# sumansamui/CMOOP_Audio_Processing

Hardware: AMD Instinct MI355X
Metric: candidate-net evals/hour (pop=40, GSC-v2) (higher is better)
Workload: dtype f32

## Files before the change

cmoop_audio_processing_amd/csrc/gemm.hip:

```cpp
#include "kernels.h"
#include <hip/hip_ext.h>
#include <cstdlib>
#include <mutex>
#include <string>
#include <type_traits>

namespace cmoop {

typedef __bf16 bf16x8 __attribute__((ext_vector_type(8)));
typedef unsigned u32x4 __attribute__((ext_vector_type(4)));

typedef __bf16 bf16x2 __attribute__((ext_vector_type(2)));

template <int NP>
__device__ __forceinline__ void split_pair(const float x, const float y, unsigned (&w)[NP]) {
    if constexpr (NP == 1) {
        w[0] = __builtin_bit_cast(unsigned, __builtin_convertvector((f32x2){x, y}, bf16x2));
    } else {
        const unsigned ux = __float_as_uint(x), uy = __float_as_uint(y);
        w[0] = __builtin_amdgcn_perm(uy, ux, 0x07060302u);
        const float rx = x - __uint_as_float(ux & 0xFFFF0000u), ry = y - __uint_as_float(uy & 0xFFFF0000u);
        const unsigned vx = __float_as_uint(rx), vy = __float_as_uint(ry);
        w[1] = __builtin_amdgcn_perm(vy, vx, 0x07060302u);
        const float sx = rx - __uint_as_float(vx & 0xFFFF0000u), sy = ry - __uint_as_float(vy & 0xFFFF0000u);
// ... 493 lines not shown
        for (int c = cbeg; c < nchunks; ++c) {
            const int buf = (c - cbeg) & 1;
            if (c + 1 < nchunks) load_chunk(c + 1, ra0, rb0);
            compute(buf);
            if (c + 1 < nchunks) store_chunk(buf ^ 1, ra0, rb0);
            __syncthreads();
        }
    }

    const int N = g.Cout;
    if (pslab) {
#pragma unroll
        for (int rt = 0; rt < RT; ++rt)
#pragma unroll
            for (int r = 0; r < 4; ++r)
#pragma unroll
                for (int ct = 0; ct < CT; ++ct)
                    pslab[(wrow + rt * 16 + q * 4 + r) * BN + wcol + ct * 16 + lr] = acc[rt][ct][r];
        continue;
    }
    if (slab) {
        float* Pz = slab + (size_t)blockIdx.z * g.M * N;
#pragma unroll
        for (int rt = 0; rt < RT; ++rt)
#pragma unroll
            for (int r = 0; r < 4; ++r) {
                const int row = m0 + wrow + rt * 16 + q * 4 + r;
                if (row >= g.M) continue;
#pragma unroll
                for (int ct = 0; ct < CT; ++ct) {
                    const int col = n0 + wcol + ct * 16 + lr;
                    if (col < N) Pz[(size_t)row * N + col] = acc[rt][ct][r];
                }
            }
        continue;
    }
    float csum[CT], csq[CT], bias_v[CT];
#pragma unroll
    for (int ct = 0; ct < CT; ++ct) {
        csum[ct] = 0.f; csq[ct] = 0.f;
        const int col = n0 + wcol + ct * 16 + lr;
        bias_v[ct] = (e.bias && col < N) ? e.bias[col] : 0.f;
    }
    const bool whole = m0 + BM <= g.M && (N % BN) == 0 && e.out_stride == 1;
    const uint32_t e_lane = (uint32_t)((m0 + wrow + q * 4) * N + n0 + wcol + lr) * 4u;
    const __amdgpu_buffer_rsrc_t yrs = __builtin_amdgcn_make_buffer_rsrc(Y, 0, g.M * N * 4, 0x00020000);
    if (whole && !e.dropout && !e.mask && !e.accumulate) {
        auto store_all = [&](auto relu_c, auto stats_c) {
#pragma unroll
            for (int rt = 0; rt < RT; ++rt)
#pragma unroll
                for (int r = 0; r < 4; ++r) {
                    const int soff = (rt * 16 + r) * N * 4;
#pragma unroll
                    for (int ct = 0; ct < CT; ++ct) {
                        float v = acc[rt][ct][r] + bias_v[ct];
                        if constexpr (decltype(relu_c)::value) v = fmaxf(v, 0.f);
                        __builtin_amdgcn_raw_buffer_store_b32(__float_as_uint(v), yrs, (int)(e_lane + ct * 64), soff, 0);
                        if constexpr (decltype(stats_c)::value) { csum[ct] += v; csq[ct] += v * v; }
                    }
                }
        };
        using T1 = std::integral_constant<bool, true>;
        using T0 = std::integral_constant<bool, false>;
        if (e.relu) { if (e.stats) store_all(T1{}, T1{}); else store_all(T1{}, T0{}); }
        else        { if (e.stats) store_all(T0{}, T1{}); else store_all(T0{}, T0{}); }
    } else if (whole && e.mask && !e.dropout && !e.relu && !e.bias && !e.stats) {
        const __amdgpu_buffer_rsrc_t mrs = __builtin_amdgcn_make_buffer_rsrc(const_cast<float*>(e.mask), 0, g.M * N * 4, 0x00020000);
#pragma unroll
        for (int rt = 0; rt < RT; ++rt) {
            float mk[4][CT], old[4][CT];
#pragma unroll
            for (int r = 0; r < 4; ++r)
#pragma unroll
                for (int ct = 0; ct < CT; ++ct) {
                    const int soff = (rt * 16 + r) * N * 4;
                    mk[r][ct] = __uint_as_float(__builtin_amdgcn_raw_buffer_load_b32(mrs, (int)(e_lane + ct * 64), soff, 0));
                    old[r][ct] = e.accumulate ? __uint_as_float(__builtin_amdgcn_raw_buffer_load_b32(yrs, (int)(e_lane + ct * 64), soff, 0)) : 0.f;
                }
#pragma unroll
            for (int r = 0; r < 4; ++r)
#pragma unroll
                for (int ct = 0; ct < CT; ++ct) {
                    const int soff = (rt * 16 + r) * N * 4;
                    float v = (mk[r][ct] > 0.f) ? acc[rt][ct][r] * e.mask_scale : 0.f;
                    if (e.accumulate) v += old[r][ct];
                    __builtin_amdgcn_raw_buffer_store_b32(__float_as_uint(v), yrs, (int)(e_lane + ct * 64), soff, 0);
                }
        }
    } else {
#pragma unroll
    for (int rt = 0; rt < RT; ++rt) {
#pragma unroll
        for (int r = 0; r < 4; ++r) {
            const int row = m0 + wrow + rt * 16 + q * 4 + r;
            if (row >= g.M) continue;
            size_t rbase;
            if (e.out_stride == 1) {
                rbase = (size_t)row * N;
            } else {
                int b = row / g.OHW, rr = row - b * g.OHW;
                int oh = rr / g.OW, ow = rr - oh * g.OW;
                rbase = ((size_t)(b * e.OHf + oh * e.out_stride) * e.OWf + ow * e.out_stride) * N;
            }
#pragma unroll
            for (int ct = 0; ct < CT; ++ct) {
                const int col = n0 + wcol + ct * 16 + lr;
                if (col >= N) continue;
                float v = acc[rt][ct][r] + bias_v[ct];
                if (e.relu) v = fmaxf(v, 0.f);
                const size_t off = rbase + col;
                if (e.dropout) {
                    uint32_t u24 = fmix32(e.drop_prefix ^ (uint32_t)((size_t)row * N + col)) >> 8;
                    v = (u24 >= e.drop_thr) ? v * e.drop_scale : 0.f;
                }
                if (e.mask) v = (e.mask[off] > 0.f) ? v * e.mask_scale : 0.f;
                if (e.accumulate) v += Y[off];
                Y[off] = v;
                csum[ct] += v;
                csq[ct] += v * v;
            }
        }
    }
    }
    if (e.stats) {
        float* red = PLANES ? reinterpret_cast<float*>(&Ah[0][0]) : &As[0][0];
#pragma unroll
        for (int ct = 0; ct < CT; ++ct) {
            csum[ct] += __shfl_xor(csum[ct], 16, 64);
            csq[ct] += __shfl_xor(csq[ct], 16, 64);
            csum[ct] += __shfl_xor(csum[ct], 32, 64);
            csq[ct] += __shfl_xor(csq[ct], 32, 64);
            if (q == 0) {
                const int c = wcol + ct * 16 + lr;
                red[((wave / WN) * BN + c) * 2] = csum[ct];
                red[((wave / WN) * BN + c) * 2 + 1] = csq[ct];
            }
        }
        __syncthreads();
        if (t < BN && n0 + t < N) {
            float a = 0.f, b = 0.f;
#pragma unroll
            for (int w = 0; w < WM; ++w) { a += red[(w * BN + t) * 2]; b += red[(w * BN + t) * 2 + 1]; }
            e.stats[((size_t)mtile * 2) * N + n0 + t] = a;
            e.stats[((size_t)mtile * 2 + 1) * N + n0 + t] = b;
        }
    }
    }
}

struct HaloDev {
    int WP, rows_max, VH;
    uint32_t wp_magic, wp_shift, vh_magic, vh_shift;
};
__host__ __device__ constexpr int halo_nst(int bm) { return bm == 256 ? 11 : 9; }
static bool halo_geometry(const ConvGeom& cg, HaloDev* hd, size_t* lds_bytes);
static size_t halo_balanced_slab_floats(const ConvGeom& cg, int* L_out);

template <int KS, int BM, int BN, int WM, bool BAL = false>
__global__ __launch_bounds__(256, 2) void halo_fwd_kernel(const float* __restrict__ X, const float* __restrict__ Wt,
                                                          float* __restrict__ Y, GeomDev g, EpiDev e, HaloDev h,
                                                          float* __restrict__ slab) {
    constexpr int WN = 4 / WM, RT = BM / WM / 16, CT = BN / WN / 16, R = KS / 2, T = KS * KS;
    constexpr int PITCH = 24;
    constexpr int NST = halo_nst(BM);
    static_assert(RT >= 1 && CT >= 1, "tile too small for the wave layout");
    extern __shared__ __attribute__((aligned(16))) float halo[];

    const int t = threadIdx.x;
    const int ncc = g.Cin >> 4;
    const int upt = ncc * KS;
    int u = 0, uend = 1;
    if constexpr (BAL) {
        const int U = ((g.M + BM - 1) / BM) * ((g.Cout + BN - 1) / BN) * upt;
        u = blockIdx.x * e.bal_L;
        uend = min(U, u + e.bal_L);
    }
    while (u < uend) {
    int mtile, ntile, c_lo = 0, c_hi = upt;
    float* pslab = nullptr;
    if constexpr (BAL) {
        const int nt = (g.Cout + BN - 1) / BN;
        const int t0 = u / upt;
        c_lo = u - t0 * upt;
        c_hi = min(upt, c_lo + (uend - u));
        mtile = t0 / nt; ntile = t0 - mtile * nt;
        const int seg = c_lo == 0 ? 0 : (int)blockIdx.x - (t0 * upt) / e.bal_L;
        pslab = slab + ((size_t)t0 * e.bal_segmax + seg) * (BM * BN);
        u += c_hi - c_lo;
        __syncthreads();
    } else {
        u = uend;
        mtile = blockIdx.x;
        const int nwg = gridDim.x, xcd = mtile & 7, idx = mtile >> 3;
        const int qn = nwg >> 3, rn = nwg & 7;
        mtile = (xcd < rn ? xcd * (qn + 1) : rn * (qn + 1) + (xcd - rn) * qn) + idx;
        ntile = blockIdx.y;
    }
    const int m0 = mtile * BM, n0 = ntile * BN;
    const int wave = t >> 6, lane = t & 63, lr = lane & 15, q = lane >> 4;
    const int wrow = (wave / WN) * (BM / WM), wcol = (wave % WN) * (BN / WN);

    auto vrow = [&](int m, int& x) {
        const int b = fastdiv(m, g.ohw_magic, g.ohw_shift), r = m - b * g.OHW;
        const int y = fastdiv(r, g.ow_magic, g.ow_shift);
        x = r - y * g.OW;
        return b * h.VH + y;
    };
    int xdummy;
    const int vbase = vrow(m0, xdummy);
    const int vlast = vrow(min(m0 + BM, g.M) - 1, xdummy);
    const int items = (vlast - vbase + 1 + 2 * R) * h.WP * 4;

    const __amdgpu_buffer_rsrc_t xr = __builtin_amdgcn_make_buffer_rsrc(
        const_cast<float*>(X), 0, (int)((uint32_t)g.B * g.H * g.W << g.cshift) * 4, 0x00020000);
    const __amdgpu_buffer_rsrc_t wr = __builtin_amdgcn_make_buffer_rsrc(const_cast<float*>(Wt), 0, g.Cout * g.K * 4, 0x00020000);
    uint32_t s_voff[NST];
#pragma unroll
    for (int it = 0; it < NST; ++it) {
        const int i = t + 256 * it, pix = i >> 2, j = i & 3;
        const int hy = fastdiv(pix, h.wp_magic, h.wp_shift), hx = pix - hy * h.WP;
        const int v = vbase - R + hy, vc = max(v, 0);
        const int b = fastdiv(vc, h.vh_magic, h.vh_shift), y = vc - b * h.VH;
        const bool ok = i < items && v >= 0 && b < g.B && y < g.H && hx >= R && hx < g.W + R;
        s_voff[it] = ok ? (uint32_t)(((((b * g.H + y) * g.W + hx - R) << g.cshift) + 4 * j) * 4) : 0xFFFFFFFFu;
    }
    float* const st_dst = halo + (t >> 2) * PITCH + (t & 3) * 4;
    f32x4 st[NST];
    auto stage_load = [&](int cc) {
#pragma unroll
        for (int it = 0; it < NST; ++it)
            st[it] = __builtin_bit_cast(f32x4, __builtin_amdgcn_raw_buffer_load_b128(xr, (int)s_voff[it], cc * 64, 0));
    };
    auto stage_store = [&]() {
#pragma unroll
        for (int it = 0; it < NST; ++it)
            if (t + 256 * it < items) *reinterpret_cast<f32x4*>(st_dst + it * 64 * PITCH) = st[it];
    };

    const float* a_ptr[RT];
#pragma unroll
    for (int rt = 0; rt < RT; ++rt) {
        int x;
        const int v = vrow(min(m0 + wrow + rt * 16 + lr, g.M - 1), x);
        a_ptr[rt] = halo + ((v - vbase) * h.WP + x) * PITCH + 4 * q;
    }
    uint32_t b_voff[CT];
#pragma unroll
    for (int ct = 0; ct < CT; ++ct) {
        const int col = n0 + wcol + ct * 16 + lr;
        b_voff[ct] = col < g.Cout ? (uint32_t)(col * g.K + 4 * q) * 4u : 0xFFFFFFFFu;
    }
    const int wp_f = h.WP * PITCH;
    auto load_b = [&](int cc, int tap, f32x4 (&b)[CT]) {
        const int soff = ((tap << g.cshift) + cc * 16) * 4;
#pragma unroll
        for (int ct = 0; ct < CT; ++ct)
            b[ct] = __builtin_bit_cast(f32x4, __builtin_amdgcn_raw_buffer_load_b128(wr, (int)b_voff[ct], soff, 0));
    };

    f32x4 acc[RT][CT];
#pragma unroll
    for (int i = 0; i < RT; ++i)
#pragma unroll
        for (int j = 0; j < CT; ++j) acc[i][j] = f32x4{0.f, 0.f, 0.f, 0.f};

    if constexpr (BAL) {
        int cc = c_lo / KS, ky = c_lo - cc * KS;
        f32x4 ac[RT], bc[CT];
        stage_load(cc);
        load_b(cc, ky * KS, bc);
        stage_store();
        __syncthreads();
#pragma unroll
        for (int rt = 0; rt < RT; ++rt) ac[rt] = *reinterpret_cast<const f32x4*>(a_ptr[rt] + ky * wp_f);
        for (int c = c_lo; c < c_hi; ++c) {
            const bool last_unit = c + 1 == c_hi, new_cc = ky == KS - 1;
            const int nky = new_cc ? 0 : ky + 1, ncc2 = new_cc ? cc + 1 : cc;
            if (new_cc && !last_unit) stage_load(cc + 1);
#pragma unroll
            for (int kx = 0; kx < KS; ++kx) {
                f32x4 an[RT], bn[CT];
#pragma unroll
                for (int ct = 0; ct < CT; ++ct) bn[ct] = bc[ct];
                if (kx + 1 < KS) {
                    load_b(cc, ky * KS + kx + 1, bn);
#pragma unroll
                    for (int rt = 0; rt < RT; ++rt)
                        an[rt] = *reinterpret_cast<const f32x4*>(a_ptr[rt] + ky * wp_f + (kx + 1) * PITCH);
                } else if (!last_unit) {
                    load_b(ncc2, nky * KS, bn);
                    if (!new_cc) {
#pragma unroll
                        for (int rt = 0; rt < RT; ++rt) an[rt] = *reinterpret_cast<const f32x4*>(a_ptr[rt] + nky * wp_f);
                    }
                }
                __builtin_amdgcn_s_setprio(1);
#pragma unroll
                for (int j = 0; j < 4; ++j)
#pragma unroll
                    for (int rt = 0; rt < RT; ++rt)
#pragma unroll
                        for (int ct = 0; ct < CT; ++ct)
                            acc[rt][ct] = __builtin_amdgcn_mfma_f32_16x16x4f32(ac[rt][j], bc[ct][j], acc[rt][ct], 0, 0, 0);
                __builtin_amdgcn_s_setprio(0);
#pragma unroll
                for (int ct = 0; ct < CT; ++ct) bc[ct] = bn[ct];
                if (kx + 1 < KS || (!last_unit && !new_cc)) {
#pragma unroll
                    for (int rt = 0; rt < RT; ++rt) ac[rt] = an[rt];
                } else if (!last_unit) {
                    __syncthreads();
                    stage_store();
                    __syncthreads();
#pragma unroll
                    for (int rt = 0; rt < RT; ++rt) ac[rt] = *reinterpret_cast<const f32x4*>(a_ptr[rt]);
                }
            }
            ky = nky; cc = ncc2;
        }
#pragma unroll
        for (int rt = 0; rt < RT; ++rt)
#pragma unroll
            for (int r = 0; r < 4; ++r)
#pragma unroll
                for (int ct = 0; ct < CT; ++ct)
                    pslab[(wrow + rt * 16 + q * 4 + r) * BN + wcol + ct * 16 + lr] = acc[rt][ct][r];
        continue;
    } else {
    f32x4 ac[RT], bc[CT];
    stage_load(0);
    load_b(0, 0, bc);
    stage_store();
    __syncthreads();
#pragma unroll
    for (int rt = 0; rt < RT; ++rt) ac[rt] = *reinterpret_cast<const f32x4*>(a_ptr[rt]);

    for (int cc = 0; cc < ncc; ++cc) {
        const bool more = cc + 1 < ncc;
#pragma unroll
        for (int tap = 0; tap < T; ++tap) {
            f32x4 an[RT], bn[CT];
#pragma unroll
            for (int ct = 0; ct < CT; ++ct) bn[ct] = bc[ct];
            if (tap + 1 < T) {
                load_b(cc, tap + 1, bn);
                const int ky = (tap + 1) / KS, kx = (tap + 1) % KS;
#pragma unroll
                for (int rt = 0; rt < RT; ++rt)
                    an[rt] = *reinterpret_cast<const f32x4*>(a_ptr[rt] + ky * wp_f + kx * PITCH);
            } else if (more) {
                load_b(cc + 1, 0, bn);
            }
            if (tap == T - 2 && more) stage_load(cc + 1);
            __builtin_amdgcn_s_setprio(1);
#pragma unroll
            for (int j = 0; j < 4; ++j)
#pragma unroll
                for (int rt = 0; rt < RT; ++rt)
#pragma unroll
                    for (int ct = 0; ct < CT; ++ct)
                        acc[rt][ct] = __builtin_amdgcn_mfma_f32_16x16x4f32(ac[rt][j], bc[ct][j], acc[rt][ct], 0, 0, 0);
            __builtin_amdgcn_s_setprio(0);
#pragma unroll
            for (int ct = 0; ct < CT; ++ct) bc[ct] = bn[ct];
            if (tap + 1 < T) {
#pragma unroll
                for (int rt = 0; rt < RT; ++rt) ac[rt] = an[rt];
            } else if (more) {
                __syncthreads();
                stage_store();
                __syncthreads();
#pragma unroll
                for (int rt = 0; rt < RT; ++rt) ac[rt] = *reinterpret_cast<const f32x4*>(a_ptr[rt]);
            }
        }
    }

    }

    const int N = g.Cout;
    float csum[CT], csq[CT], bias_v[CT];
#pragma unroll
    for (int ct = 0; ct < CT; ++ct) {
        csum[ct] = 0.f; csq[ct] = 0.f;
        const int col = n0 + wcol + ct * 16 + lr;
        bias_v[ct] = (e.bias && col < N) ? e.bias[col] : 0.f;
    }
    const bool whole = m0 + BM <= g.M && (N % BN) == 0;
    const uint32_t e_lane = (uint32_t)((m0 + wrow + q * 4) * N + n0 + wcol + lr) * 4u;
    const __amdgpu_buffer_rsrc_t yrs = __builtin_amdgcn_make_buffer_rsrc(Y, 0, g.M * N * 4, 0x00020000);
    if (whole && !e.dropout && !e.mask && !e.accumulate) {
        auto store_all = [&](auto relu_c, auto stats_c) {
#pragma unroll
            for (int rt = 0; rt < RT; ++rt)
#pragma unroll
                for (int r = 0; r < 4; ++r) {
                    const int soff = (rt * 16 + r) * N * 4;
#pragma unroll
                    for (int ct = 0; ct < CT; ++ct) {
                        float v = acc[rt][ct][r] + bias_v[ct];
                        if constexpr (decltype(relu_c)::value) v = fmaxf(v, 0.f);
                        __builtin_amdgcn_raw_buffer_store_b32(__float_as_uint(v), yrs, (int)(e_lane + ct * 64), soff, 0);
                        if constexpr (decltype(stats_c)::value) { csum[ct] += v; csq[ct] += v * v; }
                    }
                }
        };
        using T1 = std::integral_constant<bool, true>;
        using T0 = std::integral_constant<bool, false>;
        if (e.relu) { if (e.stats) store_all(T1{}, T1{}); else store_all(T1{}, T0{}); }
        else        { if (e.stats) store_all(T0{}, T1{}); else store_all(T0{}, T0{}); }
    } else if (whole && e.mask && !e.dropout && !e.relu && !e.bias && !e.stats) {
        const __amdgpu_buffer_rsrc_t mrs = __builtin_amdgcn_make_buffer_rsrc(const_cast<float*>(e.mask), 0, g.M * N * 4, 0x00020000);
#pragma unroll
        for (int rt = 0; rt < RT; ++rt) {
            float mk[4][CT], old[4][CT];
#pragma unroll
            for (int r = 0; r < 4; ++r)
#pragma unroll
                for (int ct = 0; ct < CT; ++ct) {
                    const int soff = (rt * 16 + r) * N * 4;
                    mk[r][ct] = __uint_as_float(__builtin_amdgcn_raw_buffer_load_b32(mrs, (int)(e_lane + ct * 64), soff, 0));
                    old[r][ct] = e.accumulate ? __uint_as_float(__builtin_amdgcn_raw_buffer_load_b32(yrs, (int)(e_lane + ct * 64), soff, 0)) : 0.f;
                }
#pragma unroll
            for (int r = 0; r < 4; ++r)
#pragma unroll
                for (int ct = 0; ct < CT; ++ct) {
                    const int soff = (rt * 16 + r) * N * 4;
                    float v = (mk[r][ct] > 0.f) ? acc[rt][ct][r] * e.mask_scale : 0.f;
                    if (e.accumulate) v += old[r][ct];
                    __builtin_amdgcn_raw_buffer_store_b32(__float_as_uint(v), yrs, (int)(e_lane + ct * 64), soff, 0);
                }
        }
    } else {
#pragma unroll
    for (int rt = 0; rt < RT; ++rt) {
#pragma unroll
        for (int r = 0; r < 4; ++r) {
            const int row = m0 + wrow + rt * 16 + q * 4 + r;
            if (row >= g.M) continue;
            const size_t rbase = (size_t)row * N;
#pragma unroll
            for (int ct = 0; ct < CT; ++ct) {
                const int col = n0 + wcol + ct * 16 + lr;
                if (col >= N) continue;
                float v = acc[rt][ct][r] + bias_v[ct];
                if (e.relu) v = fmaxf(v, 0.f);
                const size_t off = rbase + col;
                if (e.dropout) {
                    uint32_t u24 = fmix32(e.drop_prefix ^ (uint32_t)((size_t)row * N + col)) >> 8;
                    v = (u24 >= e.drop_thr) ? v * e.drop_scale : 0.f;
                }
                if (e.mask) v = (e.mask[off] > 0.f) ? v * e.mask_scale : 0.f;
                if (e.accumulate) v += Y[off];
                Y[off] = v;
                csum[ct] += v;
                csq[ct] += v * v;
            }
        }
    }
    }
    if (e.stats) {
        __syncthreads();
        float* red = halo;
#pragma unroll
        for (int ct = 0; ct < CT; ++ct) {
            csum[ct] += __shfl_xor(csum[ct], 16, 64);
            csq[ct] += __shfl_xor(csq[ct], 16, 64);
            csum[ct] += __shfl_xor(csum[ct], 32, 64);
            csq[ct] += __shfl_xor(csq[ct], 32, 64);
            if (q == 0) {
                const int c = wcol + ct * 16 + lr;
                red[((wave / WN) * BN + c) * 2] = csum[ct];
                red[((wave / WN) * BN + c) * 2 + 1] = csq[ct];
            }
        }
        __syncthreads();
        if (t < BN && n0 + t < N) {
            float a = 0.f, b = 0.f;
#pragma unroll
            for (int w = 0; w < WM; ++w) { a += red[(w * BN + t) * 2]; b += red[(w * BN + t) * 2 + 1]; }
            e.stats[((size_t)mtile * 2) * N + n0 + t] = a;
            e.stats[((size_t)mtile * 2 + 1) * N + n0 + t] = b;
        }
    }
    }
}

struct BalDev { int bm, bn, nt, chunks, L, segmax; };

template <int VEC>
__global__ __launch_bounds__(256) void splitk_combine_kernel(const float* __restrict__ P, float* __restrict__ Y, GeomDev g,
                                                             EpiDev e, int splits, BalDev bal) {
    const int N = g.Cout;
    const size_t total = (size_t)g.M * N;
    for (size_t i = ((size_t)blockIdx.x * 256 + threadIdx.x) * VEC; i < total; i += (size_t)gridDim.x * 256 * VEC) {
        const int row = (int)(i / N), col = (int)(i - (size_t)row * N);
        float v[VEC];
#pragma unroll
        for (int j = 0; j < VEC; ++j) v[j] = 0.f;
        if (bal.L > 0) {
            const int mt = row / bal.bm, ntl = col / bal.bn;
            const int tile = mt * bal.nt + ntl;
            const int first = (tile * bal.chunks) / bal.L;
            const int nseg = ((tile + 1) * bal.chunks + bal.L - 1) / bal.L - first;
            const float* src = P + (size_t)tile * bal.segmax * (bal.bm * bal.bn) + (size_t)(row - mt * bal.bm) * bal.bn + (col - ntl * bal.bn);
            for (int z = 0; z < nseg; ++z) {
                if constexpr (VEC == 4) {
                    const f32x4 p = *reinterpret_cast<const f32x4*>(src + (size_t)z * (bal.bm * bal.bn));
                    v[0] += p[0]; v[1] += p[1]; v[2] += p[2]; v[3] += p[3];
                } else {
                    v[0] += src[(size_t)z * (bal.bm * bal.bn)];
                }
            }
        } else
        for (int z = 0; z < splits; ++z) {
            if constexpr (VEC == 4) {
                const f32x4 p = *reinterpret_cast<const f32x4*>(P + (size_t)z * total + i);
                v[0] += p[0]; v[1] += p[1]; v[2] += p[2]; v[3] += p[3];
            } else {
                v[0] += P[(size_t)z * total + i];
            }
        }
        size_t off = i;
        if (e.out_stride != 1) {
            int b = fastdiv(row, g.ohw_magic, g.ohw_shift), rr = row - b * g.OHW;
            int oh = fastdiv(rr, g.ow_magic, g.ow_shift), ow = rr - oh * g.OW;
            off = ((size_t)(b * e.OHf + oh * e.out_stride) * e.OWf + ow * e.out_stride) * N + col;
        }
#pragma unroll
        for (int j = 0; j < VEC; ++j) {
            float x = v[j];
            if (e.bias) x += e.bias[col + j];
            if (e.relu) x = fmaxf(x, 0.f);
            if (e.dropout) {
                uint32_t u24 = fmix32(e.drop_prefix ^ (uint32_t)(i + j)) >> 8;
                x = (u24 >= e.drop_thr) ? x * e.drop_scale : 0.f;
            }
            if (e.mask) x = (e.mask[off + j] > 0.f) ? x * e.mask_scale : 0.f;
            if (e.accumulate) x += Y[off + j];
            v[j] = x;
        }
        if constexpr (VEC == 4) *reinterpret_cast<f32x4*>(Y + off) = f32x4{v[0], v[1], v[2], v[3]};
        else Y[off] = v[0];
    }
}

template <class... KA, class... A>
static void launch_timed(void (*kernel)(KA...), dim3 grid, size_t lds, hipStream_t s, const GemmTiming* tm, A&&... args) {
    if (tm && tm->start && tm->ext) {
        hipExtLaunchKernelGGL(kernel, grid, dim3(256), (uint32_t)lds, s, tm->start, tm->stop, 0, static_cast<KA>(args)...);
    } else {
        if (tm && tm->start) CMOOP_HIP(hipEventRecord(tm->start, s));
        hipLaunchKernelGGL(kernel, grid, dim3(256), lds, s, static_cast<KA>(args)...);
        if (tm && tm->start) CMOOP_HIP(hipEventRecord(tm->stop, s));
    }
}

template <int BM, int BN, int BK, int WM, int MODE = 0>
static void launch_fwd_t(const float* X, const float* Wt, float* Y, const GeomDev& g, const EpiDev& e_in, hipStream_t s,
                         const GemmTiming* tm, float* slab, int splits, int balanced_wgs = 0, const uint2* rowtab = nullptr,
                         int tab_rows = 0) {
    EpiDev e = e_in;
    dim3 grid(cdiv(g.M, BM), cdiv(g.Cout, BN), splits);
    const int nchunks = cdiv(g.K, BK);
    int cps = cdiv(nchunks, splits);
    float* sl = splits > 1 ? slab : nullptr;
    BalDev bal{BM, BN, cdiv(g.Cout, BN), nchunks, 0, 0};
    if (balanced_wgs > 0) {
        const long units = (long)grid.x * grid.y * nchunks;
        bal.L = (int)((units + balanced_wgs - 1) / balanced_wgs);
        bal.segmax = cdiv(nchunks, bal.L) + 1;
        e.bal_L = bal.L; e.bal_segmax = bal.segmax;
        grid = dim3((unsigned)((units + bal.L - 1) / bal.L), 1, 1);
        sl = slab;
        splits = 2;
    }
    launch_timed(igemm_fwd_kernel<BM, BN, BK, WM, MODE>, grid, 0, s, tm, X, Wt, Y, g, e, sl, cps, rowtab, tab_rows);
    CMOOP_HIP(hipGetLastError());
    if (splits > 1) {
        const size_t total = (size_t)g.M * g.Cout;
        if (g.Cout % 4 == 0) {
            const unsigned gridc = (unsigned)std::min<size_t>((total / 4 + 255) / 256, 4096);
            hipLaunchKernelGGL(splitk_combine_kernel<4>, dim3(gridc), dim3(256), 0, s, slab, Y, g, e, splits, bal);
        } else {
            const unsigned gridc = (unsigned)std::min<size_t>((total + 255) / 256, 4096);
            hipLaunchKernelGGL(splitk_combine_kernel<1>, dim3(gridc), dim3(256), 0, s, slab, Y, g, e, splits, bal);
        }
        CMOOP_HIP(hipGetLastError());
    }
}

static int fill_waves(long base, int max_mult, int resident, double first_thr = 0.85) {
    for (const double thr : {first_thr, 0.85}) {
        for (int m = 1; m <= max_mult; ++m) {
            const long blocks = base * m;
            const long waves = (blocks + resident - 1) / resident;
            const double u = (double)blocks / (double)(waves * resident);
            if (blocks >= resident / 2 && u >= thr) return m;
        }
    }
    int best = 1;
    double best_u = 0.0;
    for (int m = 1; m <= max_mult; ++m) {
        const long blocks = base * m;
        const long waves = (blocks + resident - 1) / resident;
        const double u = (double)blocks / (double)(waves * resident);
        if (u > best_u) { best_u = u; best = m; }
    }
    return best;
}

static inline int resident_wgs_128(int bn) { return 256 * (bn >= 64 ? 2 : 3); }

static size_t balanced_slab_floats(int M, int N, int K, int bk, int bn, int* wgs_out) {
    if (bk != 32) return 0;
    const long tiles = (long)cdiv(M, 128) * cdiv(N, bn);
    static const int mult = [] { const char* v = std::getenv("CMOOP_BALANCED_MULT"); const int m = v ? std::atoi(v) : 1; return (m == 2 || m == 4) ? m : 1; }();
    const int chunks = cdiv(K, 32), W = resident_wgs_128(bn) * mult;
    if (tiles > W || tiles * chunks < 8l * W) return 0;
    const int L = (int)((tiles * chunks + W - 1) / W);
    if (wgs_out) *wgs_out = W;
    return (size_t)tiles * (cdiv(chunks, L) + 1) * 128 * bn;
}

static void pick_tile(int M, int N, int K, int bk, size_t ws_floats, int* bm, int* bn, int* splits, int* balanced_wgs) {
    const int bn_small = N <= 16 ? 16 : (N <= 32 ? 32 : 64);
    const int bn_big = N > 64 ? 128 : bn_small;
    *splits = 1;
    *balanced_wgs = 0;
    long blocks = (long)cdiv(M, 128) * cdiv(N, bn_big);
    const long fill = std::max(32l, (long)(384 * par_scale()));
    if (blocks >= fill) { *bm = 128; *bn = bn_big; return; }
    const int nchunks = cdiv(K, bk);
    static const bool balanced_on = [] { const char* v = std::getenv("CMOOP_BALANCED"); return !(v && v[0] == '0'); }();
    if (balanced_on) {
        int W = 0;
        const size_t need = balanced_slab_floats(M, N, K, bk, bn_big, &W);
        if (need > 0 && need <= ws_floats) { *bm = 128; *bn = bn_big; *balanced_wgs = W; return; }
    }
    if (nchunks >= (M <= 512 ? 4 : 16) && ws_floats > 0) {
        const int min_chunks = M <= 512 ? 2 : 8;
        int sp = (int)std::min<long>(cdiv((int)(1024 * par_scale()), (int)blocks), nchunks / min_chunks);
        sp = std::min(sp, 32);
        if (sp > 1) sp = fill_waves(blocks, sp, std::max(32, (int)(512 * par_scale())));
        while (sp > 1 && (size_t)sp * M * N > ws_floats) --sp;
        if (sp > 1) {
            const int cps = cdiv(nchunks, sp);
            sp = cdiv(nchunks, cps);
            *bm = 128; *bn = bn_big; *splits = sp;
            return;
        }
    }
    blocks = (long)cdiv(M, 128) * cdiv(N, bn_small);
    if (blocks >= fill) { *bm = 128; *bn = bn_small; return; }
    *bm = 64; *bn = bn_small;
}

size_t igemm_splitk_workspace(const ConvGeom& g) {
    const int M = g.M(), N = g.Cout;
    const int bn_big = N > 64 ? 128 : (N <= 16 ? 16 : (N <= 32 ? 32 : 64));
    const long blocks = (long)cdiv(M, 128) * cdiv(N, bn_big);
    if (blocks >= 384) return 0;
    const int sp = std::min(32, cdiv(1024, (int)blocks));
    return std::max(std::max((size_t)sp * M * N, balanced_slab_floats(M, N, g.K(), g.Cin % 32 == 0 ? 32 : 16, bn_big, nullptr)),
                    halo_balanced_slab_floats(g, nullptr));
}

static size_t halo_balanced_slab_floats(const ConvGeom& cg, int* L_out) {
    static const bool on = [] { const char* v = std::getenv("CMOOP_HALO_BAL"); return !(v && v[0] == '0'); }();
    if (!on || cg.Cout % 64 != 0 || !halo_geometry(cg, nullptr, nullptr)) return 0;
    const long tiles = (long)cdiv(cg.M(), 128) * (cg.Cout / 64);
    const int upt = (cg.Cin / 16) * cg.KH;
    const long units = tiles * upt;
    if (tiles >= 1024 || units < 512l * 2 * cg.KH) return 0;
    const int L = (int)((units + 511) / 512);
    if (L_out) *L_out = L;
    return (size_t)tiles * (cdiv(upt, L) + 1) * 128 * 64;
}

struct FwdChoice {
    int mode, bm, bn, splits, balanced_wgs, flags;
    bool bk32_tile, use_dma, stats, halo;
    int ks, halo_L;
    int code() const { return mode * 100000000 + bm * 100000 + bn * 100 + (halo ? ks + (halo_L > 0 ? 50 : 0) : (bk32_tile ? 32 : 16)); }
};

static inline int halo_bm(int cout) { return cout >= 64 ? 128 : 256; }
static bool halo_geometry(const ConvGeom& cg, HaloDev* hd, size_t* lds_bytes) {
    const int ks = cg.KH, R = ks / 2;
    if (cg.KH != cg.KW || (ks != 3 && ks != 5) || cg.stride != 1 || cg.OH != cg.H || cg.OW != cg.W) return false;
    if (cg.pad_t != R || cg.pad_l != R || cg.Cin % 16 != 0) return false;
    if (cg.Cout % 64 != 0 && cg.Cout != 32 && cg.Cout != 16) return false;
    const int bm = halo_bm(cg.Cout);
    const int wp = (cg.W + ks - 1 + 7) / 8 * 8;
    const int span = (bm - 2 + cg.W) / cg.W + 1 + ((bm - 1) / (cg.H * cg.W) + 1) * R;
    const int rows = span + 2 * R;
    if (rows * wp * 4 > halo_nst(bm) * 256) return false;
    const size_t lds = (size_t)rows * wp * 24 * sizeof(float);
    if (lds > 64 * 1024) return false;
    if (hd) {
        hd->WP = wp; hd->rows_max = rows; hd->VH = cg.H + R;
        fastdiv_init(wp, &hd->wp_magic, &hd->wp_shift);
        fastdiv_init(cg.H + R, &hd->vh_magic, &hd->vh_shift);
    }
    if (lds_bytes) *lds_bytes = lds;
    return true;
}

void halo_rows_bound_and_need(const ConvGeom& cg, int* bound, int* need, int* items_cap) {
    HaloDev hd;
    size_t lds = 0;
    *bound = *need = *items_cap = 0;
    if (!halo_geometry(cg, &hd, &lds)) return;
    const int R = cg.KH / 2, bm = halo_bm(cg.Cout), M = cg.M(), VH = cg.H + R;
    auto vrow = [&](int m) { const int b = m / (cg.H * cg.W), r = m - b * cg.H * cg.W; return b * VH + r / cg.W; };
    int worst = 0;
    for (int m0 = 0; m0 < M; m0 += bm) worst = std::max(worst, vrow(std::min(m0 + bm, M) - 1) - vrow(m0) + 1 + 2 * R);
    *bound = hd.rows_max; *need = worst; *items_cap = halo_nst(bm) * 256 / (hd.WP * 4);
}

static size_t halo_lds_for_occupancy(size_t lds, long wgs, int occ_env) {
    auto fill = [&](long slots) { return (double)wgs / (double)(((wgs + slots - 1) / slots) * slots); };
    const bool better = wgs <= 1536 && fill(512) > fill(768) + 0.05;
    const bool two = occ_env < 0 ? better : (occ_env == 2 || (occ_env != 3 && lds <= 53 * 1024 && better));
    return two ? std::max(lds, (size_t)55 * 1024) : lds;
}

static FwdChoice choose_fwd(const ConvGeom& cg, const GemmEpilogue& ep, size_t ws_floats, bool want_stats, bool have_rowtab) {
    FwdChoice c;
    const int M = cg.M(), N = cg.Cout, K = cg.K();
    c.mode = resolve_mode(ep.mode);
    const bool bk32 = c.mode != GEMM_FP32 || (cg.Cin % 32 == 0);
    pick_tile(M, N, K, bk32 ? 32 : 16, ws_floats, &c.bm, &c.bn, &c.splits, &c.balanced_wgs);
    c.stats = want_stats && c.splits == 1 && !c.balanced_wgs && ep.out_stride == 1 && !ep.accumulate;
    c.bk32_tile = c.mode != GEMM_FP32 ||
                  (bk32 && !(c.bm == 128 && c.bn == 64 && c.splits == 1 && !c.balanced_wgs && (long)cdiv(M, 128) * cdiv(N, 64) >= 1024));
    static const int dma_env = [] { const char* v = std::getenv("CMOOP_DMA"); return v ? std::atoi(v) : 1; }();
    c.use_dma = dma_env && c.mode == GEMM_FP32 && (cg.Cin % 32 == 0) && cg.KH * cg.KW <= 32 && c.bk32_tile && c.bm == 128 && c.bn == 32;
    if (c.use_dma) c.mode = GEMM_FP32_DMA;
    const int bk = c.bk32_tile ? 32 : 16;
    static const bool halo_env = [] { const char* v = std::getenv("CMOOP_HALO"); return !(v && v[0] == '0'); }();
    c.ks = cg.KH;
    c.halo = halo_env && (c.mode == GEMM_FP32 || c.mode == GEMM_FP32_DMA) && c.bm == 128 && c.splits == 1 && !c.balanced_wgs && ep.out_stride == 1 &&
             halo_geometry(cg, nullptr, nullptr);
    c.halo_L = 0;
    if (c.halo) {
        c.mode = GEMM_FP32_HALO; c.use_dma = false;
        c.bm = halo_bm(cg.Cout);
        c.bn = std::min(cg.Cout, 64);
    } else if (halo_env && (c.mode == GEMM_FP32 || c.mode == GEMM_FP32_DMA) && c.bm == 128 && (c.splits > 1 || c.balanced_wgs) && ep.out_stride == 1) {
        int L = 0;
        const size_t need = halo_balanced_slab_floats(cg, &L);
        if (need > 0 && need <= ws_floats) {
            c.halo = true; c.halo_L = L; c.mode = GEMM_FP32_HALO; c.use_dma = false; c.stats = false;
            c.bm = 128; c.bn = 64; c.splits = 1; c.balanced_wgs = 512;
        }
    }
    c.flags = (c.splits > 1 ? GEMM_FLAG_SPLITK : 0) | (c.stats ? GEMM_FLAG_STATS : 0) | (c.balanced_wgs ? GEMM_FLAG_BALANCED : 0) |
              ((!c.halo && have_rowtab && (cg.Cin % bk) == 0 && cg.KH * cg.KW <= 32) ? GEMM_FLAG_ROWTAB : 0);
    return c;
}

int igemm_fwd_plan(const ConvGeom& g, const GemmEpilogue& ep, size_t ws_floats, bool want_stats, bool have_rowtab, int* flags_out) {
    igemm_check_range(g);
    CMOOP_REQUIRE(ilog2_exact(g.Cin) >= 4, "implicit GEMM needs C_in a power of two >= 16");
    const FwdChoice c = choose_fwd(g, ep, ws_floats, want_stats, have_rowtab);
    if (flags_out) *flags_out = c.flags;
    return c.code();
}

int launch_igemm_fwd(const float* X, const float* Wt, float* Y, const ConvGeom& cg, const GemmEpilogue& ep,
                     hipStream_t s, const GemmTiming* tm, float* splitk_ws, size_t splitk_ws_floats, int* stats_blocks,
                     const void* rowtab_v, int tab_rows, int* flags_out) {
    if (stats_blocks) *stats_blocks = 0;
    if (flags_out) *flags_out = 0;
    const uint2* rowtab = static_cast<const uint2*>(rowtab_v);
    GeomDev g = to_dev(cg);
    if (g.M == 0) return 0;
    EpiDev e;
    e.bias = ep.bias; e.mask = ep.mask; e.mask_scale = ep.mask_scale; e.relu = ep.relu;
    e.accumulate = ep.accumulate; e.out_stride = ep.out_stride; e.OHf = ep.OHf; e.OWf = ep.OWf;
    e.dropout = ep.dropout; e.drop_prefix = ep.drop_prefix; e.drop_thr = ep.drop_thr; e.drop_scale = ep.drop_scale;
    if (e.out_stride > 1)
        CMOOP_REQUIRE((int64_t)g.B * e.OHf * e.OWf * g.Cout < (1ll << 29), "scattered output too large");
    const FwdChoice ch = choose_fwd(cg, ep, splitk_ws ? splitk_ws_floats : 0, ep.stats != nullptr && stats_blocks != nullptr, rowtab != nullptr);
    const int mode = ch.mode == GEMM_FP32_DMA ? (int)GEMM_FP32 : ch.mode;
    const int bm = ch.bm, bn = ch.bn, splits = ch.splits, balanced_wgs = ch.balanced_wgs;
    const bool bk32_tile = ch.bk32_tile, use_dma = ch.use_dma;
    e.bal_L = 0; e.bal_segmax = 0;
    e.stats = ch.stats ? ep.stats : nullptr;
    if (e.stats) *stats_blocks = cdiv(g.M, bm);
    if (flags_out) *flags_out = ch.flags;
    if (ch.halo) {
        HaloDev hd;
        size_t lds = 0;
        CMOOP_REQUIRE(halo_geometry(cg, &hd, &lds), "halo kernel chosen for a geometry it does not accept");
        dim3 grid(cdiv(g.M, bm), cdiv(g.Cout, bn));
        BalDev bal{bm, bn, cdiv(g.Cout, bn), (cg.Cin / 16) * cg.KH, ch.halo_L, 0};
        if (ch.halo_L > 0) {
            bal.segmax = cdiv(bal.chunks, bal.L) + 1;
            e.bal_L = bal.L; e.bal_segmax = bal.segmax;
            const long units = (long)grid.x * grid.y * bal.chunks;
            grid = dim3((unsigned)((units + bal.L - 1) / bal.L), 1, 1);
            lds = std::max(lds, (size_t)55 * 1024);
        }
        static const int occ_env = [] { const char* v = std::getenv("CMOOP_HALO_OCC"); const int o = v ? std::atoi(v) : 0; return o == 2 || o == 3 ? o : 0; }();
        lds = halo_lds_for_occupancy(lds, (long)grid.x * grid.y, occ_env);
        auto run = [&](auto kernel) { launch_timed(kernel, grid, lds, s, tm, X, Wt, Y, g, e, hd, splitk_ws); };
#define CMOOP_HALO_KS(KS_)                                                                     \
        do {                                                                                   \
            if (ch.halo_L > 0) run(halo_fwd_kernel<KS_, 128, 64, 2, true>);                    \
            else if (bn == 64) run(halo_fwd_kernel<KS_, 128, 64, 2, false>);                   \
            else if (bn == 32) run(halo_fwd_kernel<KS_, 256, 32, 4, false>);                   \
            else run(halo_fwd_kernel<KS_, 256, 16, 4, false>);                                 \
        } while (0)
        if (cg.KH == 5) CMOOP_HALO_KS(5); else CMOOP_HALO_KS(3);
#undef CMOOP_HALO_KS
        CMOOP_HIP(hipGetLastError());
        if (ch.halo_L > 0) {
            const size_t total = (size_t)g.M * g.Cout;
            const unsigned gridc = (unsigned)std::min<size_t>((total / 4 + 255) / 256, 4096);
            hipLaunchKernelGGL(splitk_combine_kernel<4>, dim3(gridc), dim3(256), 0, s, splitk_ws, Y, g, e, 2, bal);
            CMOOP_HIP(hipGetLastError());
        }
        return ch.code();
    }
#define CMOOP_FWD(BM_, BN_, WM_)                                                              \
    do {                                                                                      \
        if (mode == GEMM_BF16X3) launch_fwd_t<BM_, BN_, 32, WM_, GEMM_BF16X3>(X, Wt, Y, g, e, s, tm, splitk_ws, splits, balanced_wgs, rowtab, tab_rows);   \
        else if (mode == GEMM_BF16) launch_fwd_t<BM_, BN_, 32, WM_, GEMM_BF16>(X, Wt, Y, g, e, s, tm, splitk_ws, splits, balanced_wgs, rowtab, tab_rows);  \
        else if (use_dma && BM_ == 128 && BN_ == 32) launch_fwd_t<BM_, 32, 32, WM_, GEMM_FP32_DMA>(X, Wt, Y, g, e, s, tm, splitk_ws, splits, balanced_wgs, rowtab, tab_rows);   \
        else if (bk32_tile) launch_fwd_t<BM_, BN_, 32, WM_>(X, Wt, Y, g, e, s, tm, splitk_ws, splits, balanced_wgs, rowtab, tab_rows);   \
        else launch_fwd_t<BM_, BN_, 16, WM_>(X, Wt, Y, g, e, s, tm, splitk_ws, splits, 0, rowtab, tab_rows);        \
    } while (0)
    if (bm == 128) {
        if (bn == 128) CMOOP_FWD(128, 128, 2);
        else if (bn == 64) CMOOP_FWD(128, 64, 4);
        else if (bn == 32) CMOOP_FWD(128, 32, 4);
        else CMOOP_FWD(128, 16, 4);
    } else {
        if (bn == 64) CMOOP_FWD(64, 64, 2);
        else if (bn == 32) CMOOP_FWD(64, 32, 4);
        else CMOOP_FWD(64, 16, 4);
    }
#undef CMOOP_FWD
    return ch.code();
}

__global__ __launch_bounds__(256) void build_rowtab_kernel(GeomDev g, uint2* __restrict__ tab, int rows_padded) {
    const int m = blockIdx.x * 256 + threadIdx.x;
    if (m >= rows_padded) return;
    if (m >= g.M) { tab[m] = make_uint2(0u, 0xFFFFFFFFu); return; }
    const int b = fastdiv(m, g.ohw_magic, g.ohw_shift), r = m - b * g.OHW;
    const int oh = fastdiv(r, g.ow_magic, g.ow_shift), ow = r - oh * g.OW;
    const int ih0 = oh * g.stride - g.pad_t, iw0 = ow * g.stride - g.pad_l;
    const int hlo = max(0, -ih0), hhi = min(g.KH, g.H - ih0);
    const int wlo = max(0, -iw0), whi = min(g.KW, g.W - iw0);
    const uint32_t wmask = (whi > wlo) ? (((1u << whi) - 1u) & ~((1u << wlo) - 1u)) : 0u;
    uint32_t okm = 0;
    for (int kh = 0; kh < g.KH; ++kh)
        if (kh >= hlo && kh < hhi) okm |= wmask << (kh * g.KW);
    const uint32_t bias = (uint32_t)((g.pad_t * g.W + g.pad_l) << g.cshift);
    tab[m] = make_uint2(((uint32_t)(((b * g.H + ih0) * g.W + iw0) << g.cshift) + bias) * 4u, ~okm);
}

int rowtab_rows(const ConvGeom& g) { return cdiv(g.M(), 256) * 256; }

void launch_build_rowtab(const ConvGeom& cg, void* tab, hipStream_t s) {
    GeomDev g = to_dev(cg);
    CMOOP_REQUIRE(g.KH * g.KW <= 32, "row table: at most 32 filter taps");
    const int rows = rowtab_rows(cg);
    if (rows == 0) return;
    hipLaunchKernelGGL(build_rowtab_kernel, dim3(cdiv(rows, 256)), dim3(256), 0, s, g, static_cast<uint2*>(tab), rows);
    CMOOP_HIP(hipGetLastError());
}

template <int BCO, int BKI, int MC = 32>
__global__ __launch_bounds__(256) void igemm_wgrad_kernel(const float* __restrict__ X, const float* __restrict__ dY,
                                                          float* __restrict__ P, GeomDev g, int rows_per_slice,
                                                          float* __restrict__ Pbias, size_t slab_stride,
                                                          const uint2* __restrict__ rowtab, int tab_rows, int grouped_kt,
                                                          int grouped_ct, int grouped_slices) {
    constexpr int NBUF = MC == 32 ? 2 : 1;
    constexpr int LDX = BKI + 16;
    constexpr int LDY = (BCO == 16) ? 16 : BCO + 16;
    constexpr int CT = BCO / 16, KT = BKI / 16;
    constexpr int WC = CT >= 4 ? 2 : CT;
    constexpr int WK = 4 / WC;
    constexpr int CPW = CT / WC, KPW = KT / WK;
    constexpr int TPRX = BKI / 4, RPPX = 256 / TPRX, XPASS = MC / RPPX;
    constexpr int TPRY = BCO / 4, RPPY = 256 / TPRY;
    constexpr int YPASS = (MC + RPPY - 1) / RPPY;
    __shared__ __attribute__((aligned(16))) float Xs[NBUF][MC * LDX];
    __shared__ __attribute__((aligned(16))) float Ys[NBUF][MC * LDY];

    const int t = threadIdx.x;
    int bx = blockIdx.x, by = blockIdx.y, bz = blockIdx.z;
    if (grouped_kt > 0) {
        const int L = blockIdx.x, xcd = L & 7, j = L >> 3;
        const int per = grouped_kt * grouped_ct;
        const int grp = j / per, r = j - grp * per;
        by = r / grouped_kt; bx = r - by * grouped_kt;
        bz = grp * 8 + xcd;
        if (bz >= grouped_slices) return;
    }
    const int k0 = bx * BKI, co0 = by * BCO;
    const int mbeg = bz * rows_per_slice;
    const int mend = min(g.M, mbeg + rows_per_slice);

    const int xq = t % TPRX, xrow = t / TPRX;
    const int kidx = k0 + 4 * xq;
    const bool kok = kidx < g.K;
    const int tap = kidx >> g.cshift, ci = kidx & (g.Cin - 1);
    const int kh = (tap * g.rcp_kw) >> 16, kw = tap - kh * g.KW;
    const int yq = t % TPRY, yrow = t / TPRY;
    const bool cok = (co0 + 4 * yq) < g.Cout;

    f32x4 rx[XPASS], ry[YPASS];
    const bool fast = rowtab != nullptr && (g.Cout & 3) == 0;
    const uint32_t x_bias = (uint32_t)((g.pad_t * g.W + g.pad_l) << g.cshift);
    const __amdgpu_buffer_rsrc_t xr = __builtin_amdgcn_make_buffer_rsrc(
        const_cast<float*>(X) - x_bias, 0, (int)(((uint32_t)g.B * g.H * g.W << g.cshift) + x_bias) * 4, 0x00020000);
    const __amdgpu_buffer_rsrc_t yr = __builtin_amdgcn_make_buffer_rsrc(const_cast<float*>(dY), 0, g.M * g.Cout * 4, 0x00020000);
    const __amdgpu_buffer_rsrc_t tr = __builtin_amdgcn_make_buffer_rsrc(const_cast<uint2*>(rowtab), 0, fast ? tab_rows * 8 : 0, 0x00020000);
    const uint32_t koff = (uint32_t)((((kh * g.W + kw) << g.cshift) + ci) * 4);
    const uint32_t kdead = kok ? 0u : 0xFFFFFFFFu;
    uint32_t y_voff[YPASS];
#pragma unroll
    for (int p = 0; p < YPASS; ++p) {
        const int rl = yrow + p * RPPY;
        y_voff[p] = (rl < MC && cok) ? (uint32_t)(rl * g.Cout + co0 + 4 * yq) * 4u : 0xFFFFFFF0u;
    }
    uint2 te[XPASS];
    auto load_tab = [&](int mc) {
#pragma unroll
        for (int p = 0; p < XPASS; ++p) {
            const auto v = __builtin_amdgcn_raw_buffer_load_b64(tr, (xrow + p * RPPX) * 8, mc * 8, 0);
            te[p] = make_uint2(v[0], v[1]);
        }
    };
    auto load_chunk_fast = [&](int mc) {
#pragma unroll
        for (int p = 0; p < XPASS; ++p) {
            const uint32_t dead = (uint32_t)__builtin_amdgcn_sbfe((int)te[p].y, tap, 1);
            rx[p] = __builtin_bit_cast(f32x4, __builtin_amdgcn_raw_buffer_load_b128(xr, (int)((te[p].x + koff) | dead | kdead), 0, 0));
        }
#pragma unroll
        for (int p = 0; p < YPASS; ++p)
            ry[p] = __builtin_bit_cast(f32x4, __builtin_amdgcn_raw_buffer_load_b128(yr, (int)y_voff[p], mc * g.Cout * 4, 0));
    };
    auto load_chunk = [&](int mc) {
#pragma unroll
        for (int p = 0; p < XPASS; ++p) {
            const int m = mc + xrow + p * RPPX;
            const int mm = m < mend ? m : 0;
            const int b = fastdiv(mm, g.ohw_magic, g.ohw_shift), r = mm - b * g.OHW;
            const int oh = fastdiv(r, g.ow_magic, g.ow_shift), ow = r - oh * g.OW;
            const int ih = oh * g.stride - g.pad_t + kh, iw = ow * g.stride - g.pad_l + kw;
            const bool ok = kok && m < mend && (unsigned)ih < (unsigned)g.H && (unsigned)iw < (unsigned)g.W;
            const float* src = ok ? X + (((size_t)((b * g.H + ih) * g.W + iw)) << g.cshift) + ci : g.zeros;
            rx[p] = *reinterpret_cast<const f32x4*>(src);
        }
#pragma unroll
        for (int p = 0; p < YPASS; ++p) {
            int rl = yrow + p * RPPY;
            int m = mc + rl;
            f32x4 v = {0.f, 0.f, 0.f, 0.f};
            const bool ok = rl < MC && m < mend && cok;
            if ((g.Cout & 3) == 0) {
                const float* src = ok ? dY + (size_t)m * g.Cout + co0 + 4 * yq : g.zeros;
                v = *reinterpret_cast<const f32x4*>(src);
            } else if (ok) {
                const float* src = dY + (size_t)m * g.Cout + co0 + 4 * yq;
#pragma unroll
                for (int j = 0; j < 4; ++j)
// ... 664 lines not shown
```

Measured before the change: 440.0.

## Store balanced halo partials lane-major and reduce them in a tile-aware combine kernel

```diff
diff --git a/cmoop_audio_processing_amd/csrc/gemm.hip b/cmoop_audio_processing_amd/csrc/gemm.hip
--- a/cmoop_audio_processing_amd/csrc/gemm.hip
+++ b/cmoop_audio_processing_amd/csrc/gemm.hip
@@ -669,6 +669,7 @@
 struct HaloDev {
     int WP, rows_max, VH;
     uint32_t wp_magic, wp_shift, vh_magic, vh_shift;
+    int lane_major;
 };
 __host__ __device__ constexpr int halo_nst(int bm) { return bm == 256 ? 11 : 9; }
 static bool halo_geometry(const ConvGeom& cg, HaloDev* hd, size_t* lds_bytes);
@@ -836,6 +837,14 @@
             }
             ky = nky; cc = ncc2;
         }
+        if (h.lane_major) {
+#pragma unroll
+            for (int rt = 0; rt < RT; ++rt)
+#pragma unroll
+                for (int ct = 0; ct < CT; ++ct)
+                    *reinterpret_cast<f32x4*>(pslab + ((rt * CT + ct) * 256 + t) * 4) = acc[rt][ct];
+            continue;
+        }
 #pragma unroll
         for (int rt = 0; rt < RT; ++rt)
 #pragma unroll
@@ -896,88 +905,7 @@
 
     }
 
-    const int N = g.Cout;
-    float csum[CT], csq[CT], bias_v[CT];
-#pragma unroll
-    for (int ct = 0; ct < CT; ++ct) {
-        csum[ct] = 0.f; csq[ct] = 0.f;
-        const int col = n0 + wcol + ct * 16 + lr;
-        bias_v[ct] = (e.bias && col < N) ? e.bias[col] : 0.f;
-    }
-    const bool whole = m0 + BM <= g.M && (N % BN) == 0;
-    const uint32_t e_lane = (uint32_t)((m0 + wrow + q * 4) * N + n0 + wcol + lr) * 4u;
-    const __amdgpu_buffer_rsrc_t yrs = __builtin_amdgcn_make_buffer_rsrc(Y, 0, g.M * N * 4, 0x00020000);
-    if (whole && !e.dropout && !e.mask && !e.accumulate) {
-        auto store_all = [&](auto relu_c, auto stats_c) {
-#pragma unroll
-            for (int rt = 0; rt < RT; ++rt)
-#pragma unroll
-                for (int r = 0; r < 4; ++r) {
-                    const int soff = (rt * 16 + r) * N * 4;
-#pragma unroll
-                    for (int ct = 0; ct < CT; ++ct) {
-                        float v = acc[rt][ct][r] + bias_v[ct];
-                        if constexpr (decltype(relu_c)::value) v = fmaxf(v, 0.f);
-                        __builtin_amdgcn_raw_buffer_store_b32(__float_as_uint(v), yrs, (int)(e_lane + ct * 64), soff, 0);
-                        if constexpr (decltype(stats_c)::value) { csum[ct] += v; csq[ct] += v * v; }
-                    }
-                }
-        };
-        using T1 = std::integral_constant<bool, true>;
-        using T0 = std::integral_constant<bool, false>;
-        if (e.relu) { if (e.stats) store_all(T1{}, T1{}); else store_all(T1{}, T0{}); }
-        else        { if (e.stats) store_all(T0{}, T1{}); else store_all(T0{}, T0{}); }
-    } else if (whole && e.mask && !e.dropout && !e.relu && !e.bias && !e.stats) {
-        const __amdgpu_buffer_rsrc_t mrs = __builtin_amdgcn_make_buffer_rsrc(const_cast<float*>(e.mask), 0, g.M * N * 4, 0x00020000);
-#pragma unroll
-        for (int rt = 0; rt < RT; ++rt) {
-            float mk[4][CT], old[4][CT];
-#pragma unroll
-            for (int r = 0; r < 4; ++r)
-#pragma unroll
-                for (int ct = 0; ct < CT; ++ct) {
-                    const int soff = (rt * 16 + r) * N * 4;
-                    mk[r][ct] = __uint_as_float(__builtin_amdgcn_raw_buffer_load_b32(mrs, (int)(e_lane + ct * 64), soff, 0));
-                    old[r][ct] = e.accumulate ? __uint_as_float(__builtin_amdgcn_raw_buffer_load_b32(yrs, (int)(e_lane + ct * 64), soff, 0)) : 0.f;
-                }
-#pragma unroll
-            for (int r = 0; r < 4; ++r)
-#pragma unroll
-                for (int ct = 0; ct < CT; ++ct) {
-                    const int soff = (rt * 16 + r) * N * 4;
-                    float v = (mk[r][ct] > 0.f) ? acc[rt][ct][r] * e.mask_scale : 0.f;
-                    if (e.accumulate) v += old[r][ct];
-                    __builtin_amdgcn_raw_buffer_store_b32(__float_as_uint(v), yrs, (int)(e_lane + ct * 64), soff, 0);
-                }
-        }
-    } else {
-#pragma unroll
-    for (int rt = 0; rt < RT; ++rt) {
-#pragma unroll
-        for (int r = 0; r < 4; ++r) {
-            const int row = m0 + wrow + rt * 16 + q * 4 + r;
-            if (row >= g.M) continue;
-            const size_t rbase = (size_t)row * N;
-#pragma unroll
-            for (int ct = 0; ct < CT; ++ct) {
-                const int col = n0 + wcol + ct * 16 + lr;
-                if (col >= N) continue;
-                float v = acc[rt][ct][r] + bias_v[ct];
-                if (e.relu) v = fmaxf(v, 0.f);
-                const size_t off = rbase + col;
-                if (e.dropout) {
-                    uint32_t u24 = fmix32(e.drop_prefix ^ (uint32_t)((size_t)row * N + col)) >> 8;
-                    v = (u24 >= e.drop_thr) ? v * e.drop_scale : 0.f;
-                }
-                if (e.mask) v = (e.mask[off] > 0.f) ? v * e.mask_scale : 0.f;
-                if (e.accumulate) v += Y[off];
-                Y[off] = v;
-                csum[ct] += v;
-                csq[ct] += v * v;
-            }
-        }
-    }
-    }
+#include "halo_epilogue.inc"
     if (e.stats) {
         __syncthreads();
         float* red = halo;
@@ -1062,6 +990,47 @@
         if constexpr (VEC == 4) *reinterpret_cast<f32x4*>(Y + off) = f32x4{v[0], v[1], v[2], v[3]};
         else Y[off] = v[0];
     }
+}
+
+template <int BM, int BN, int WM>
+__global__ __launch_bounds__(256) void halo_combine_kernel(const float* __restrict__ P, float* __restrict__ Y, GeomDev g,
+                                                           EpiDev e_in, BalDev bal) {
+    EpiDev e = e_in;
+    e.stats = nullptr;
+    constexpr int WN = 4 / WM, RT = BM / WM / 16, CT = BN / WN / 16;
+    const int t = threadIdx.x, wave = t >> 6, lane = t & 63;
+    const int tile = blockIdx.x;
+    const int mtile = tile / bal.nt, ntile = tile - mtile * bal.nt;
+    const int first = (tile * bal.chunks) / bal.L;
+    const int nseg = ((tile + 1) * bal.chunks + bal.L - 1) / bal.L - first;
+    const float* src = P + (size_t)tile * bal.segmax * (BM * BN) + t * 4;
+    f32x4 acc[RT][CT];
+#pragma unroll
+    for (int i = 0; i < RT; ++i)
+#pragma unroll
+        for (int j = 0; j < CT; ++j) acc[i][j] = f32x4{0.f, 0.f, 0.f, 0.f};
+    for (int z = 0; z < nseg; z += 2) {
+        const bool two = z + 1 < nseg;
+        f32x4 p[RT][CT], p2[RT][CT];
+#pragma unroll
+        for (int rt = 0; rt < RT; ++rt)
+#pragma unroll
+            for (int ct = 0; ct < CT; ++ct) {
+                const float* a = src + (size_t)z * (BM * BN) + (rt * CT + ct) * 1024;
+                p[rt][ct] = *reinterpret_cast<const f32x4*>(a);
+                p2[rt][ct] = two ? *reinterpret_cast<const f32x4*>(a + BM * BN) : f32x4{0.f, 0.f, 0.f, 0.f};
+            }
+#pragma unroll
+        for (int rt = 0; rt < RT; ++rt)
+#pragma unroll
+            for (int ct = 0; ct < CT; ++ct) {
+                acc[rt][ct] += p[rt][ct];
+                if (two) acc[rt][ct] += p2[rt][ct];
+            }
+    }
+    const int m0 = mtile * BM, n0 = ntile * BN, lr = lane & 15, q = lane >> 4;
+    const int wrow = (wave / WN) * (BM / WM), wcol = (wave % WN) * (BN / WN);
+#include "halo_epilogue.inc"
 }
 
 template <class... KA, class... A>
@@ -1218,7 +1187,7 @@
     const size_t lds = (size_t)rows * wp * 24 * sizeof(float);
     if (lds > 64 * 1024) return false;
     if (hd) {
-        hd->WP = wp; hd->rows_max = rows; hd->VH = cg.H + R;
+        hd->WP = wp; hd->rows_max = rows; hd->VH = cg.H + R; hd->lane_major = 0;
         fastdiv_init(wp, &hd->wp_magic, &hd->wp_shift);
         fastdiv_init(cg.H + R, &hd->vh_magic, &hd->vh_shift);
     }
@@ -1316,7 +1285,10 @@
         CMOOP_REQUIRE(halo_geometry(cg, &hd, &lds), "halo kernel chosen for a geometry it does not accept");
         dim3 grid(cdiv(g.M, bm), cdiv(g.Cout, bn));
         BalDev bal{bm, bn, cdiv(g.Cout, bn), (cg.Cin / 16) * cg.KH, ch.halo_L, 0};
+        static const bool slab_lanes = [] { const char* v = std::getenv("CMOOP_HALO_SLAB"); return !(v && v[0] == '0'); }();
         if (ch.halo_L > 0) {
+            CMOOP_REQUIRE(e.out_stride == 1, "balanced halo launch: the combine writes a dense output");
+            hd.lane_major = slab_lanes ? 1 : 0;
             bal.segmax = cdiv(bal.chunks, bal.L) + 1;
             e.bal_L = bal.L; e.bal_segmax = bal.segmax;
             const long units = (long)grid.x * grid.y * bal.chunks;
@@ -1337,9 +1309,13 @@
 #undef CMOOP_HALO_KS
         CMOOP_HIP(hipGetLastError());
         if (ch.halo_L > 0) {
-            const size_t total = (size_t)g.M * g.Cout;
-            const unsigned gridc = (unsigned)std::min<size_t>((total / 4 + 255) / 256, 4096);
-            hipLaunchKernelGGL(splitk_combine_kernel<4>, dim3(gridc), dim3(256), 0, s, splitk_ws, Y, g, e, 2, bal);
+            if (hd.lane_major) {
+                hipLaunchKernelGGL((halo_combine_kernel<128, 64, 2>), dim3(cdiv(g.M, bm) * bal.nt), dim3(256), 0, s, splitk_ws, Y, g, e, bal);
+            } else {
+                const size_t total = (size_t)g.M * g.Cout;
+                const unsigned gridc = (unsigned)std::min<size_t>((total / 4 + 255) / 256, 4096);
+                hipLaunchKernelGGL(splitk_combine_kernel<4>, dim3(gridc), dim3(256), 0, s, splitk_ws, Y, g, e, 2, bal);
+            }
             CMOOP_HIP(hipGetLastError());
         }
         return ch.code();
diff --git a/cmoop_audio_processing_amd/csrc/halo_epilogue.inc b/cmoop_audio_processing_amd/csrc/halo_epilogue.inc
--- /dev/null
+++ b/cmoop_audio_processing_amd/csrc/halo_epilogue.inc
@@ -0,0 +1,82 @@
+    const int N = g.Cout;
+    float csum[CT], csq[CT], bias_v[CT];
+#pragma unroll
+    for (int ct = 0; ct < CT; ++ct) {
+        csum[ct] = 0.f; csq[ct] = 0.f;
+        const int col = n0 + wcol + ct * 16 + lr;
+        bias_v[ct] = (e.bias && col < N) ? e.bias[col] : 0.f;
+    }
+    const bool whole = m0 + BM <= g.M && (N % BN) == 0;
+    const uint32_t e_lane = (uint32_t)((m0 + wrow + q * 4) * N + n0 + wcol + lr) * 4u;
+    const __amdgpu_buffer_rsrc_t yrs = __builtin_amdgcn_make_buffer_rsrc(Y, 0, g.M * N * 4, 0x00020000);
+    if (whole && !e.dropout && !e.mask && !e.accumulate) {
+        auto store_all = [&](auto relu_c, auto stats_c) {
+#pragma unroll
+            for (int rt = 0; rt < RT; ++rt)
+#pragma unroll
+                for (int r = 0; r < 4; ++r) {
+                    const int soff = (rt * 16 + r) * N * 4;
+#pragma unroll
+                    for (int ct = 0; ct < CT; ++ct) {
+                        float v = acc[rt][ct][r] + bias_v[ct];
+                        if constexpr (decltype(relu_c)::value) v = fmaxf(v, 0.f);
+                        __builtin_amdgcn_raw_buffer_store_b32(__float_as_uint(v), yrs, (int)(e_lane + ct * 64), soff, 0);
+                        if constexpr (decltype(stats_c)::value) { csum[ct] += v; csq[ct] += v * v; }
+                    }
+                }
+        };
+        using T1 = std::integral_constant<bool, true>;
+        using T0 = std::integral_constant<bool, false>;
+        if (e.relu) { if (e.stats) store_all(T1{}, T1{}); else store_all(T1{}, T0{}); }
+        else        { if (e.stats) store_all(T0{}, T1{}); else store_all(T0{}, T0{}); }
+    } else if (whole && e.mask && !e.dropout && !e.relu && !e.bias && !e.stats) {
+        const __amdgpu_buffer_rsrc_t mrs = __builtin_amdgcn_make_buffer_rsrc(const_cast<float*>(e.mask), 0, g.M * N * 4, 0x00020000);
+#pragma unroll
+        for (int rt = 0; rt < RT; ++rt) {
+            float mk[4][CT], old[4][CT];
+#pragma unroll
+            for (int r = 0; r < 4; ++r)
+#pragma unroll
+                for (int ct = 0; ct < CT; ++ct) {
+                    const int soff = (rt * 16 + r) * N * 4;
+                    mk[r][ct] = __uint_as_float(__builtin_amdgcn_raw_buffer_load_b32(mrs, (int)(e_lane + ct * 64), soff, 0));
+                    old[r][ct] = e.accumulate ? __uint_as_float(__builtin_amdgcn_raw_buffer_load_b32(yrs, (int)(e_lane + ct * 64), soff, 0)) : 0.f;
+                }
+#pragma unroll
+            for (int r = 0; r < 4; ++r)
+#pragma unroll
+                for (int ct = 0; ct < CT; ++ct) {
+                    const int soff = (rt * 16 + r) * N * 4;
+                    float v = (mk[r][ct] > 0.f) ? acc[rt][ct][r] * e.mask_scale : 0.f;
+                    if (e.accumulate) v += old[r][ct];
+                    __builtin_amdgcn_raw_buffer_store_b32(__float_as_uint(v), yrs, (int)(e_lane + ct * 64), soff, 0);
+                }
+        }
+    } else {
+#pragma unroll
+    for (int rt = 0; rt < RT; ++rt) {
+#pragma unroll
+        for (int r = 0; r < 4; ++r) {
+            const int row = m0 + wrow + rt * 16 + q * 4 + r;
+            if (row >= g.M) continue;
+            const size_t rbase = (size_t)row * N;
+#pragma unroll
+            for (int ct = 0; ct < CT; ++ct) {
+                const int col = n0 + wcol + ct * 16 + lr;
+                if (col >= N) continue;
+                float v = acc[rt][ct][r] + bias_v[ct];
+                if (e.relu) v = fmaxf(v, 0.f);
+                const size_t off = rbase + col;
+                if (e.dropout) {
+                    uint32_t u24 = fmix32(e.drop_prefix ^ (uint32_t)((size_t)row * N + col)) >> 8;
+                    v = (u24 >= e.drop_thr) ? v * e.drop_scale : 0.f;
+                }
+                if (e.mask) v = (e.mask[off] > 0.f) ? v * e.mask_scale : 0.f;
+                if (e.accumulate) v += Y[off];
+                Y[off] = v;
+                csum[ct] += v;
+                csq[ct] += v * v;
+            }
+        }
+    }
+    }
```

After: 443.5, median of 6. Within noise of the previous version (+0.8%).
